# ProfessorNova/PPO-Car

Measured on AMD Instinct MI355X. Metric: env steps/sec (whole node) on big_track.json, 16 rays, higher is better.
Workload: dtype f32

## Files before the change

### include/ppocar.h

```cpp
#ifndef PPOCAR_H
#define PPOCAR_H

#include <stdint.h>

#ifdef __cplusplus
extern "C" {
#endif

#define PC_OK 0
#define PC_ERR_INVALID_ARG (-1)
#define PC_ERR_IO (-2)
#define PC_ERR_PARSE (-3)
#define PC_ERR_HIP (-4)
#define PC_ERR_UNSUPPORTED (-5)
#define PC_ERR_NO_DEVICE (-6)
#define PC_ERR_TIMEOUT (-7)

#define PC_DTYPE_F32 0
#define PC_DTYPE_F64 1

typedef struct pc_track pc_track;
typedef struct pc_env pc_env;
typedef struct pc_policy pc_policy;
typedef struct pc_xchg pc_xchg;
// ... 87 lines not shown
                         uint64_t offset, const uint64_t* offset_dev, float* obs_buf, float* act_buf, float* rew_buf, float* val_buf,
                         float* term_buf, float* trunc_buf, float* logprob_buf, float* next_obs, float* next_term, float* next_trunc,
                         float* last_value, float* reward_sum, float* final_obs, int64_t slots, void* stream);

int pc_ppo_gather(int device, const int64_t* idx, int B, int D, const float* obs, const float* act, const float* logprob,
                  const float* adv, const float* ret, float* o_obs, float* o_act, float* o_logprob, float* o_adv, float* o_ret,
                  void* stream);
int pc_ppo_loss(int device, const float* logits, const float* values, const float* act, const float* old_logprob,
                const float* adv, const float* ret, int B, int A, double clip_ratio, double vf_coef, double ent_coef,
                float* dlogits, float* dvalues, float* metrics, void* stream);
int pc_clip_adam(int device, float* param, float* grad, float* exp_avg, float* exp_avg_sq, float* step_count, const float* lr_dev,
                 int64_t n, double max_norm, double grad_scale, double beta1, double beta2, double eps, void* stream);
int pc_clip_adam_advanced(int device, float* param, const float* grad, float* exp_avg, float* exp_avg_sq, const float* step_count,
                          const float* lr_dev, int64_t n, double max_norm, double grad_scale, double beta1, double beta2, double eps,
                          void* stream);

int64_t pc_ppo_workspace_floats(int B, int D, int H, int A);
int pc_ppo_minibatch(int device, const int64_t* idx, int B, int D, int H, int A, const float* obs, const float* act,
                     const float* old_logprob, const float* adv, const float* ret, float* param, float* grad, float* exp_avg,
                     float* exp_avg_sq, float* step_count, const float* lr_dev, double clip_ratio, double vf_coef, double ent_coef,
                     double max_norm, double beta1, double beta2, double eps, float* metrics, float* workspace, int apply,
                     void* stream);

int64_t pc_ppo_prepared_floats(int B, int D);
int pc_ppo_prepare(int device, const int64_t* idx, int64_t idx_ld, int n_mb, int B, int D, const float* obs, const float* act,
                   const float* old_logprob, const float* adv, const float* ret, float* prepared, void* stream);
int pc_ppo_minibatch_prepared(int device, const float* prepared_mb, int B, int D, int H, int A, float* param, float* grad, float* exp_avg,
                              float* exp_avg_sq, float* step_count, const float* lr_dev, double clip_ratio, double vf_coef,
                              double ent_coef, double max_norm, double beta1, double beta2, double eps, float* metrics,
                              float* workspace, int apply, void* stream);


#define PC_DIAG_FLOATS 8
int64_t pc_ppo_diag_workspace_floats(int B, int D, int H, int A);
int pc_ppo_minibatch_diag(int device, const int64_t* idx, int B, int D, int H, int A, const float* obs, const float* act,
                          const float* old_logprob, const float* adv, const float* ret, float* param, float* grad, float* exp_avg,
                          float* exp_avg_sq, float* step_count, const float* lr_dev, double clip_ratio, double vf_coef, double ent_coef,
                          double max_norm, double beta1, double beta2, double eps, float* metrics, float* workspace, int apply,
                          float* diag, double target_kl, void* stream);
int pc_ppo_minibatch_prepared_diag(int device, const float* prepared_mb, int B, int D, int H, int A, float* param, float* grad, float* exp_avg,
                                   float* exp_avg_sq, float* step_count, const float* lr_dev, double clip_ratio, double vf_coef,
                                   double ent_coef, double max_norm, double beta1, double beta2, double eps, float* metrics,
                                   float* workspace, int apply, float* diag, double target_kl, void* stream);
int pc_ppo_loss_diag(int device, const float* logits, const float* values, const float* act, const float* old_logprob,
                     const float* adv, const float* ret, int B, int A, double clip_ratio, double vf_coef, double ent_coef,
                     float* dlogits, float* dvalues, float* metrics, float* diag, double target_kl, void* stream);
// ... 45 lines not shown
```

### ppo-car_amd/_capi.py

```python
import ctypes as C
import os

import torch

_HERE = os.path.dirname(os.path.abspath(__file__))
_LIB_PATH = os.path.join(_HERE, "libppocar.so")

PC_OK = 0
PC_ERR_INVALID_ARG, PC_ERR_IO, PC_ERR_PARSE, PC_ERR_HIP, PC_ERR_UNSUPPORTED, PC_ERR_NO_DEVICE, PC_ERR_TIMEOUT = -1, -2, -3, -4, -5, -6, -7
PC_XCHG_HANDLE_BYTES = 128
PC_DTYPE_F32, PC_DTYPE_F64 = 0, 1
PC_EPISODE_BUFFER, PC_EPISODE_STEPS = 0, 1
PC_DIAG_FLOATS = 8
PC_TIME_LIMIT = 1000
PC_OPT_ROLLOUT_FORM, PC_OPT_ROLLOUT_EPW, PC_OPT_ROLLOUT_FAST = 1, 2, 3
PC_KERNEL_NAMES = {0: "none", 1: "K9", 2: "K9s", 3: "K9-literal", 4: "K9d-filter", 5: "K9s-literal", 6: "K9d-selector", 7: "K9m", 8: "K9m-literal"}
PC_STEP_NAMES = {0: "none", 1: "K1", 2: "K1f", 3: "K1f-table"}
DTYPES = {"f32": PC_DTYPE_F32, "float32": PC_DTYPE_F32, "f64": PC_DTYPE_F64, "float64": PC_DTYPE_F64}


class PpoCarError(RuntimeError):
    def __init__(self, code, what):
        self.code = code
        msg = f"{what}: {lib.pc_strerror(code).decode()} (code {code})"
# ... 48 lines not shown
    "pc_build_ablate": (_i, []),
    "pc_env_get_state": (_i, [_vp] * 9),
    "pc_env_set_state": (_i, [_vp] * 9),
    "pc_gae": (_i, [_i, _vp, _vp, _vp, _vp, _vp, _vp, _vp, _d, _d, _i64, _i64, _vp, _vp, _vp]),
    "pc_episode_stats": (_i, [_i, _vp, _vp, _vp, _vp, _vp, _i64, _i64, _i, _d, _vp, _vp, _vp]),
    "pc_gae_episodes": (_i, [_i, _vp, _vp, _vp, _vp, _vp, _vp, _vp, _d, _d, _i64, _i64, _vp, _vp, _d, _vp, _vp, _vp]),
    "pc_gae_bootstrap": (_i, [_i, _vp, _vp, _vp, _vp, _vp, _vp, _vp, _vp, _i64, _d, _d, _i64, _i64, _vp, _vp, _d, _vp, _vp, _vp]),
    "pc_sample": (_i, [_i, _vp, _i64, _i, C.c_uint64, C.c_uint64, _vp, _vp, _vp, _vp]),
    "pc_policy_create": (_i, [_i, _i, _i, _i, _i, _i, C.POINTER(_vp)]),
    "pc_policy_destroy": (None, [_vp]),
    "pc_policy_get": (_i, [_vp, C.POINTER(_i), C.POINTER(_i), C.POINTER(_i64)]),
    "pc_policy_pack": (_i, [_vp] + [_vp] * 8 + [_vp, _vp]),
    "pc_policy_pack_checked": (_i, [_vp] + [_vp] * 8 + [_vp, _vp, _vp]),
    "pc_policy_act": (_i, [_vp, _vp, _i64, _vp, C.c_uint64, C.c_uint64, _vp] + [_vp] * 5 + [_vp]),
    "pc_rollout": (_i, [_vp, _vp, _vp, _i64, _d, C.c_uint64, C.c_uint64, _vp] + [_vp] * 12 + [_vp]),
    "pc_rollout_final_obs": (_i, [_vp, _vp, _vp, _i64, _d, C.c_uint64, C.c_uint64, _vp] + [_vp] * 12 + [_vp, _i64, _vp]),
    "pc_env_set_option": (_i, [_vp, _i, _i]),
    "pc_env_get_option": (_i, [_vp, _i, C.POINTER(_i)]),
    "pc_ppo_gather": (_i, [_i, _vp, _i, _i] + [_vp] * 10 + [_vp]),
    "pc_ppo_loss": (_i, [_i] + [_vp] * 6 + [_i, _i, _d, _d, _d, _vp, _vp, _vp, _vp]),
    "pc_clip_adam": (_i, [_i] + [_vp] * 6 + [_i64, _d, _d, _d, _d, _d, _vp]),
    "pc_clip_adam_advanced": (_i, [_i] + [_vp] * 6 + [_i64, _d, _d, _d, _d, _d, _vp]),
    "pc_ppo_workspace_floats": (_i64, [_i, _i, _i, _i]),
    "pc_ppo_prepared_floats": (_i64, [_i, _i]),
    "pc_ppo_prepare": (_i, [_i, _vp, _i64, _i, _i, _i] + [_vp] * 5 + [_vp, _vp]),
    "pc_ppo_minibatch_prepared": (_i, [_i, _vp, _i, _i, _i, _i] + [_vp] * 6 + [_d] * 7 + [_vp, _vp, _i, _vp]),
    "pc_ppo_epoch_state_floats": (_i64, [_i, _i, _i]),
    "pc_ppo_epoch_prepared": (_i, [_i, _vp, _i, _i, _i, _i, _i] + [_vp] * 6 + [_d] * 7 + [_vp, _vp, _vp, _vp]),
    "pc_ppo_minibatch": (_i, [_i, _vp, _i, _i, _i, _i] + [_vp] * 5 + [_vp] * 6 + [_d] * 7 + [_vp, _vp, _i, _vp]),
    "pc_ppo_diag_workspace_floats": (_i64, [_i, _i, _i, _i]),
    "pc_ppo_minibatch_diag": (_i, [_i, _vp, _i, _i, _i, _i] + [_vp] * 5 + [_vp] * 6 + [_d] * 7 + [_vp, _vp, _i, _vp, _d, _vp]),
    "pc_ppo_minibatch_prepared_diag": (_i, [_i, _vp, _i, _i, _i, _i] + [_vp] * 6 + [_d] * 7 + [_vp, _vp, _i, _vp, _d, _vp]),
    "pc_ppo_loss_diag": (_i, [_i] + [_vp] * 6 + [_i, _i, _d, _d, _d, _vp, _vp, _vp, _vp, _d, _vp]),
    "pc_clip_adam_diag": (_i, [_i] + [_vp] * 6 + [_i64, _d, _d, _d, _d, _d, _vp, _vp]),
    "pc_explained_variance_workspace_doubles": (_i64, [_i]),
    "pc_explained_variance": (_i, [_i, _vp, _vp, _i64, _vp, _vp, _vp]),
    "pc_xchg_create": (_i, [_i, _i, _i, _i64, C.POINTER(_vp)]),
    "pc_xchg_local_handle": (_i, [_vp, _vp]),
    "pc_xchg_connect": (_i, [_vp, _vp]),
    "pc_xchg_connect_local": (_i, [_vp, _vp]),
    "pc_xchg_allreduce_group": (_i, [_vp, _vp, _vp]),
    "pc_xchg_set_timeout": (_i, [_vp, _d]),
    "pc_xchg_allreduce": (_i, [_vp, _vp, _vp]),
    "pc_xchg_status": (_i, [_vp]),
    "pc_xchg_destroy": (None, [_vp]),
    "pc_strerror": (C.c_char_p, [_i]),
# ... 21 lines not shown
```

### ppo-car_amd/csrc/kernels/update.hpp

```cpp
#pragma once

__global__ __launch_bounds__(256) void ppo_gather_kernel(const int64_t* __restrict__ idx, const int B, const int D,
                                                         const float* __restrict__ obs, const float* __restrict__ act,
                                                         const float* __restrict__ logprob, const float* __restrict__ adv,
                                                         const float* __restrict__ ret, float* __restrict__ o_obs,
                                                         float* __restrict__ o_act, float* __restrict__ o_logprob,
                                                         float* __restrict__ o_adv, float* __restrict__ o_ret) {
    const int W = D + 4;
    const int i = blockIdx.x * blockDim.x + threadIdx.x;
    if (i >= B * W) return;
    const int b = i / W, c = i - b * W;
    const int64_t src = idx[b];
    if (c < D) o_obs[b * D + c] = obs[src * D + c];
    else if (c == D) o_act[b] = act[src];
    else if (c == D + 1) o_logprob[b] = logprob[src];
    else if (c == D + 2) o_adv[b] = adv[src];
    else o_ret[b] = ret[src];
}

__device__ __forceinline__ float block_sum(float v, float* sh) {
    for (int m = 32; m >= 1; m >>= 1) v += __shfl_xor(v, m, 64);
    const int w = threadIdx.x >> 6, nw = (blockDim.x + 63) >> 6;
    __syncthreads();
    if ((threadIdx.x & 63) == 0) sh[w] = v;
// ... 208 lines not shown

constexpr int FB_S = 8;

struct AdamCoef { float coef, step_size, bc2_sqrt, beta1, beta2, eps; };
__device__ __forceinline__ AdamCoef adam_coef(const float norm_sq, const float step, const float lr, const float max_norm, const float beta1,
                                              const float beta2, const float eps) {
    AdamCoef c;
    c.coef = fminf(max_norm / (sqrtf(norm_sq) + 1e-6f), 1.0f);
    const float bc1 = 1.0f - powf(beta1, step), bc2 = 1.0f - powf(beta2, step);
    c.step_size = lr / bc1;
    c.bc2_sqrt = sqrtf(bc2);
    c.beta1 = beta1;
    c.beta2 = beta2;
    c.eps = eps;
    return c;
}
__device__ __forceinline__ void adam_elem(const AdamCoef& c, const float g_raw, float& p, float& m, float& v) {
    const float g = g_raw * c.coef;
    m = m + (1.0f - c.beta1) * (g - m);
    v = c.beta2 * v + (1.0f - c.beta2) * g * g;
    const float denom = sqrtf(v) / c.bc2_sqrt + c.eps;
    p = p - c.step_size * (m / denom);
}
__device__ __forceinline__ float norm_sq_from_partials(const float* __restrict__ norm_partial, const int n_norm) {
    float ss = 0.0f;
    for (int j = 0; j < n_norm; ++j) ss += norm_partial[j];
    return ss;
}
struct AdamDefer {
    const float* __restrict__ grad;
    const float* __restrict__ m_in;
    const float* __restrict__ v_in;
    float* __restrict__ p_out;
    float* __restrict__ m_out;
    float* __restrict__ v_out;
    const float* __restrict__ norm_partial;
    int n_norm;
    const float* __restrict__ step_count;
    const float* __restrict__ lr_dev;
    float max_norm, beta1, beta2, eps;
};

__device__ __forceinline__ float wave_sum(float v) {
#define PC_DPP(ctrl, rmask) v += __builtin_bit_cast(float, __builtin_amdgcn_update_dpp(0, __builtin_bit_cast(int, v), ctrl, rmask, 0xf, false))
    PC_DPP(0x111, 0xf);
    PC_DPP(0x112, 0xf);
    PC_DPP(0x114, 0xf);
    PC_DPP(0x118, 0xf);
    PC_DPP(0x142, 0xa);
    PC_DPP(0x143, 0xc);
#undef PC_DPP
    return __builtin_bit_cast(float, __builtin_amdgcn_readlane(__builtin_bit_cast(int, v), 63));
}

__device__ __forceinline__ void adv_stats(const float (&a_loc)[4], const float a_sum, const int B, float* sh, float& mean, float& sd) {
    const int u = threadIdx.x;
    mean = block_sum(a_sum, sh) * (1.0f / (float)B);
    float d2 = 0.0f;
#pragma unroll
    for (int j = 0; j < 4; ++j) {
        const int i = u + j * 256;
        const float dv = i < B ? a_loc[j] - mean : 0.0f;
        d2 += dv * dv;
    }
    sd = fmaxf(sqrtf(block_sum(d2, sh) / (float)(B - 1)), 1e-5f);
}

__global__ __launch_bounds__(256) void ppo_prepare_kernel(const int64_t* __restrict__ idx, const int64_t idx_ld, const int B, const int D,
                                                          const float* __restrict__ obs, const float* __restrict__ act,
                                                          const float* __restrict__ old_lp, const float* __restrict__ adv,
                                                          const float* __restrict__ ret, float* __restrict__ prepared,
                                                          const int64_t prep_ld) {
    __shared__ float sh[16];
    const int u = threadIdx.x;
    const int64_t* ix = idx + (int64_t)blockIdx.x * idx_ld;
    float* out = prepared + (int64_t)blockIdx.x * prep_ld;
    float* ps = out + (size_t)B * D;
    float a_loc[4], a_sum = 0.0f;
#pragma unroll
    for (int j = 0; j < 4; ++j) {
        const int i = u + j * 256;
        const int64_t src = i < B ? ix[i] : 0;
        a_loc[j] = i < B ? adv[src] : 0.0f;
        a_sum += a_loc[j];
        if (i < B) {
            ps[i] = act[src];
            ps[B + i] = old_lp[src];
            ps[2 * B + i] = a_loc[j];
            ps[3 * B + i] = ret[src];
        }
    }
    for (int i = u; i < B * D; i += 256) {
        const int b = i / D, f = i - b * D;
        out[i] = obs[ix[b] * D + f];
    }
    float mean, sd;
    adv_stats(a_loc, a_sum, B, sh, mean, sd);
    if (u == 0) {
        ps[4 * B] = mean;
        ps[4 * B + 1] = sd;
        ps[4 * B + 2] = 0.0f;
        ps[4 * B + 3] = 0.0f;
    }
}

template <int DMAX, int AC = 0, int DC = 0, bool DEFER = false, bool DIAG = false>
__device__ __forceinline__ void ppo_fwdbwd_body(const int wg, const int64_t* __restrict__ idx, const int B, const int D_rt, const int A_rt,
                                                const float* __restrict__ obs, const float* __restrict__ act,
                                                const float* __restrict__ old_lp, const float* __restrict__ adv,
                                                const float* __restrict__ ret, const float* __restrict__ param,
                                                const float clip, const float vf, const float ec,
                                                float* __restrict__ partial, float* __restrict__ metric_partial,
                                                const float* __restrict__ prep, const AdamDefer df,
                                                const float* __restrict__ diag = nullptr, float* __restrict__ diag_partial = nullptr) {
    constexpr int H = 256, S = FB_S, LDT = DMAX + 1, LDH = H + 1;
    static_assert(!(DIAG && DEFER), "the deferred chain has no diagnostics form");
    if constexpr (DIAG) if (diag[4] != 0.0f) return;
// ... 6 lines not shown
    __shared__ float sMet[S][DIAG ? 5 : 3];
    __shared__ float sSmp[S][4];
    __shared__ __attribute__((aligned(16))) float sT[H * LDT > 2 * S * LDH + 16 * LDH + 4 * S * 16 ? H * LDT : 2 * S * LDH + 16 * LDH + 4 * S * 16];
    static_assert(H * LDT >= H * DMAX + 8, "the tile holds one [H][D] block in natural order plus an alignment shift");
    float* sHid = sT;
    float* sW2 = sT + 2 * S * LDH;
    float* sP2 = sW2 + 16 * LDH;
    const int u = threadIdx.x;
    PC_STAMP_U(0)
    __syncthreads();
    const int o_aW1 = 0, o_ab1 = H * D, o_aW2 = o_ab1 + H, o_ab2 = o_aW2 + A * H, o_cW1 = o_ab2 + A, o_cb1 = o_cW1 + H * D,
              o_cW2 = o_cb1 + H, o_cb2 = o_cW2 + H, n_param = o_cb2 + 1;

    const int s0 = wg * S;
    int64_t my_src = 0;
    int64_t a_src[4] = {0, 0, 0, 0};
    if (!prep) {
        if (u < S && s0 + u < B) my_src = idx[s0 + u];
#pragma unroll
        for (int j = 0; j < 4; ++j) a_src[j] = u + j * 256 < B ? idx[u + j * 256] : 0;
    }
    const bool defer = DEFER && df.grad != nullptr;
    const bool wr = defer && wg == 0;
    float w2a[16], w2a_g[16], w2a_m[16], w2a_v[16];
#pragma unroll
    for (int o = 0; o < 16; ++o) {
        w2a[o] = o < A ? param[o_aW2 + o * H + u] : 0.0f;
        w2a_g[o] = w2a_m[o] = w2a_v[o] = 0.0f;
        if (defer && o < A) {
            w2a_g[o] = df.grad[o_aW2 + o * H + u];
            w2a_m[o] = df.m_in[o_aW2 + o * H + u];
            w2a_v[o] = df.v_in[o_aW2 + o * H + u];
        }
    }
    float w2c = param[o_cW2 + u], b1a = param[o_ab1 + u], b1c = param[o_cb1 + u];
    const int ob = u & 15;
    const int o_b2 = ob < A ? o_ab2 + ob : o_cb2;
    float b2 = ob <= A ? param[o_b2] : 0.0f;
    float sc_g[4] = {0.0f, 0.0f, 0.0f, 0.0f}, sc_m[4] = {0.0f, 0.0f, 0.0f, 0.0f}, sc_v[4] = {0.0f, 0.0f, 0.0f, 0.0f};
    const int sc_i[4] = {o_cW2 + u, o_ab1 + u, o_cb1 + u, o_b2};
    if (defer) {
#pragma unroll
        for (int q = 0; q < 4; ++q) {
            if (q < 3 || ob <= A) {
                sc_g[q] = df.grad[sc_i[q]];
                sc_m[q] = df.m_in[sc_i[q]];
// ... 8 lines not shown
#pragma unroll
    for (int net = 0; net < 2; ++net) {
        const int off = net == 0 ? o_aW1 : o_cW1, b4 = off & ~3;
        w1_shift[net] = off - b4;
        w1_b4[net] = b4;
        w1_n4[net] = (off + H * D - b4 + 3) >> 2;
        const f32x4* __restrict__ src = reinterpret_cast<const f32x4*>(param + b4);
#pragma unroll
        for (int j = 0; j < NV4; ++j) {
            const int i4 = u + 256 * j;
            const f32x4 z = {0.0f, 0.0f, 0.0f, 0.0f};
            w1raw4[net][j] = i4 < w1_n4[net] ? src[i4] : z;
            if constexpr (DEFER) {
                w1g[net][j] = w1m[net][j] = w1v[net][j] = z;
                if (defer && i4 < w1_n4[net]) {
                    w1g[net][j] = reinterpret_cast<const f32x4*>(df.grad + b4)[i4];
                    w1m[net][j] = reinterpret_cast<const f32x4*>(df.m_in + b4)[i4];
                    w1v[net][j] = reinterpret_cast<const f32x4*>(df.v_in + b4)[i4];
                }
            }
        }
    }
    if constexpr (DEFER) if (defer) {
        const AdamCoef ac = adam_coef(norm_sq_from_partials(df.norm_partial, df.n_norm), df.step_count[0], df.lr_dev[0], df.max_norm, df.beta1,
                                      df.beta2, df.eps);
#pragma unroll
        for (int o = 0; o < 16; ++o) {
            if (o < A) {
                adam_elem(ac, w2a_g[o], w2a[o], w2a_m[o], w2a_v[o]);
                if (wr) {
                    df.p_out[o_aW2 + o * H + u] = w2a[o];
                    df.m_out[o_aW2 + o * H + u] = w2a_m[o];
                    df.v_out[o_aW2 + o * H + u] = w2a_v[o];
                }
            }
        }
        float sc_p[4] = {w2c, b1a, b1c, b2};
#pragma unroll
        for (int q = 0; q < 4; ++q) {
            if (q < 3 || ob <= A) {
                adam_elem(ac, sc_g[q], sc_p[q], sc_m[q], sc_v[q]);
                if (wr && (q < 3 || u <= A)) {
                    df.p_out[sc_i[q]] = sc_p[q];
                    df.m_out[sc_i[q]] = sc_m[q];
                    df.v_out[sc_i[q]] = sc_v[q];
                }
            }
// ... 285 lines not shown
__global__ __launch_bounds__(256) void ppo_fwdbwd_kernel(const int64_t* __restrict__ idx, const int B, const int D, const int A,
                                                         const float* __restrict__ obs, const float* __restrict__ act,
                                                         const float* __restrict__ old_lp, const float* __restrict__ adv,
                                                         const float* __restrict__ ret, const float* __restrict__ param,
                                                         const float clip, const float vf, const float ec,
                                                         float* __restrict__ partial, float* __restrict__ metric_partial,
                                                         const float* __restrict__ prep, const AdamDefer df) {
    ppo_fwdbwd_body<DMAX, AC, DC, DEFER>(blockIdx.x, idx, B, D, A, obs, act, old_lp, adv, ret, param, clip, vf, ec, partial, metric_partial, prep, df);
}
template <int DMAX, int AC = 0, int DC = 0>
__global__ __launch_bounds__(256) void ppo_fwdbwd_diag_kernel(const int64_t* __restrict__ idx, const int B, const int D, const int A,
                                                              const float* __restrict__ obs, const float* __restrict__ act,
                                                              const float* __restrict__ old_lp, const float* __restrict__ adv,
                                                              const float* __restrict__ ret, const float* __restrict__ param,
                                                              const float clip, const float vf, const float ec,
                                                              float* __restrict__ partial, float* __restrict__ metric_partial,
                                                              const float* __restrict__ prep, const float* __restrict__ diag,
                                                              float* __restrict__ diag_partial) {
    ppo_fwdbwd_body<DMAX, AC, DC, false, true>(blockIdx.x, idx, B, D, A, obs, act, old_lp, adv, ret, param, clip, vf, ec, partial, metric_partial, prep,
                                               AdamDefer{}, diag, diag_partial);
}

template <bool DIAG = false>
__device__ __forceinline__ void grad_reduce_body(const int blk, const float* __restrict__ partial, const int n_part, const int n,
                                                          const int HD, const int mid_end, const int n_pad,
                                                          float* __restrict__ grad, float* __restrict__ norm_partial,
                                                          const float* __restrict__ metric_partial, const int B, const float vf,
                                                          const float ec, float* __restrict__ metrics, float* __restrict__ step_count,
                                                          float* __restrict__ diag = nullptr, const float* __restrict__ diag_partial = nullptr,
                                                          const float kl_stop = 0.0f) {
    __shared__ float sh[16];
    __syncthreads();
    float dg_val = 0.0f, flag_val = 0.0f;
    if constexpr (DIAG) {
        if ((int)threadIdx.x < 2 * n_part) dg_val = diag_partial[threadIdx.x];
        flag_val = diag[4];
    }
    const int i = blk * blockDim.x + threadIdx.x;
    const float mp_first = (blk == 0 && (int)threadIdx.x < n_part * 4) ? metric_partial[threadIdx.x] : 0.0f;
    float g = 0.0f;
    if (i < n) {
        const int pm = i < HD ? i : (i < mid_end ? i + HD : (i < mid_end + HD ? i - (mid_end - HD) : i));
        const float* __restrict__ pp = partial + pm;
        int pidx = 0;
        for (; pidx + 64 <= n_part; pidx += 64) {
            float t[64];
#pragma unroll
            for (int j = 0; j < 64; ++j) t[j] = pp[(size_t)(pidx + j) * n_pad];
#pragma unroll
            for (int j = 0; j < 64; ++j) g += t[j];
        }
        for (; pidx + 32 <= n_part; pidx += 32) {
            float t[32];
#pragma unroll
            for (int j = 0; j < 32; ++j) t[j] = pp[(size_t)(pidx + j) * n_pad];
#pragma unroll
            for (int j = 0; j < 32; ++j) g += t[j];
        }
        for (; pidx + 8 <= n_part; pidx += 8) {
            float t[8];
#pragma unroll
            for (int j = 0; j < 8; ++j) t[j] = pp[(size_t)(pidx + j) * n_pad];
#pragma unroll
            for (int j = 0; j < 8; ++j) g += t[j];
        }
        for (; pidx < n_part; ++pidx) g += pp[(size_t)pidx * n_pad];
    }
    if constexpr (DIAG) {
        __shared__ __attribute__((aligned(8))) float sDg[256];
        sDg[threadIdx.x] = dg_val;
        __syncthreads();
        if (flag_val != 0.0f) return;
        float kl = 0.0f, nc = 0.0f;
#pragma unroll 8
        for (int p = 0; p < n_part; ++p) {
            const float2 v = reinterpret_cast<const float2*>(sDg)[p];
            kl += v.x;
            nc += v.y;
        }
        const DiagSums d{kl / (float)B, nc / (float)B};
        if (blk == 0 && threadIdx.x == 0) diag_book(diag, d, kl_stop);
        if (kl_stop > 0.0f && d.kl > kl_stop) return;
    }
    if (i < n) grad[i] = g;
    const float ss = block_sum(g * g, sh);
    if (threadIdx.x == 0) norm_partial[blk] = ss;
    if (blk == 0) {
        __shared__ float sMp[256];
        float mt[3] = {0.0f, 0.0f, 0.0f};
        for (int p0 = 0; p0 < n_part; p0 += 64) {
            __syncthreads();
            sMp[threadIdx.x] = p0 == 0 ? mp_first : (p0 * 4 + (int)threadIdx.x < n_part * 4 ? metric_partial[p0 * 4 + threadIdx.x] : 0.0f);
            __syncthreads();
            if (threadIdx.x < 3) {
                float mv[64];
#pragma unroll
                for (int pidx = 0; pidx < 64; ++pidx) mv[pidx] = sMp[pidx * 4 + threadIdx.x];
#pragma unroll
                for (int pidx = 0; pidx < 64; ++pidx) mt[threadIdx.x] += mv[pidx];
            }
        }
        if (threadIdx.x < 3) sh[threadIdx.x] = mt[threadIdx.x] / (float)B;
        __syncthreads();
        if (threadIdx.x == 0) {
            metrics[0] += sh[0];
            metrics[1] += sh[1];
            metrics[2] += sh[2];
            metrics[3] += sh[0] + vf * sh[1] - ec * sh[2];
            if (step_count) step_count[0] += 1.0f;
        }
    }
}

__global__ __launch_bounds__(256) void grad_reduce_kernel(const float* __restrict__ partial, const int n_part, const int n,
                                                          const int HD, const int mid_end, const int n_pad,
                                                          float* __restrict__ grad, float* __restrict__ norm_partial,
                                                          const float* __restrict__ metric_partial, const int B, const float vf,
                                                          const float ec, float* __restrict__ metrics, float* __restrict__ step_count) {
    grad_reduce_body(blockIdx.x, partial, n_part, n, HD, mid_end, n_pad, grad, norm_partial, metric_partial, B, vf, ec, metrics, step_count);
}
__global__ __launch_bounds__(256) void grad_reduce_diag_kernel(const float* __restrict__ partial, const int n_part, const int n,
                                                               const int HD, const int mid_end, const int n_pad,
                                                               float* __restrict__ grad, float* __restrict__ norm_partial,
                                                               const float* __restrict__ metric_partial, const int B, const float vf,
                                                               const float ec, float* __restrict__ metrics, float* __restrict__ step_count,
                                                               float* __restrict__ diag, const float* __restrict__ diag_partial,
                                                               const float kl_stop) {
    grad_reduce_body<true>(blockIdx.x, partial, n_part, n, HD, mid_end, n_pad, grad, norm_partial, metric_partial, B, vf, ec, metrics, step_count,
                           diag, diag_partial, kl_stop);
}

template <bool DIAG = false>
__device__ __forceinline__ void adam_body(const int blk, const float* __restrict__ p_in, const float* __restrict__ m_in, const float* __restrict__ v_in,
                                          float* __restrict__ grad, float* __restrict__ p_out, float* __restrict__ m_out, float* __restrict__ v_out,
                                          const float* __restrict__ step_count, const float* __restrict__ lr_dev,
                                          const float* __restrict__ norm_partial, const int n_norm, const int n, const float max_norm,
                                          const float beta1, const float beta2, const float eps, const float* __restrict__ diag = nullptr) {
    __shared__ float sNorm[256];
    const int i = blk * blockDim.x + threadIdx.x;
    const bool live = i < n;
    const float g_raw = live ? grad[i] : 0.0f;
    float m = live ? m_in[i] : 0.0f, v = live ? v_in[i] : 0.0f, p = live ? p_in[i] : 0.0f;
    const float step = step_count[0], lr = lr_dev[0];
    float flag = 0.0f;
    if constexpr (DIAG) flag = diag[4];
    float ss = 0.0f;
    for (int j0 = 0; j0 < n_norm; j0 += 256) {
        __syncthreads();
        if (j0 + (int)threadIdx.x < n_norm) sNorm[threadIdx.x] = norm_partial[j0 + threadIdx.x];
        __syncthreads();
        const int cnt = n_norm - j0 < 256 ? n_norm - j0 : 256;
        for (int j = 0; j < cnt; ++j) ss += sNorm[j];
    }
    const AdamCoef ac = adam_coef(ss, step, lr, max_norm, beta1, beta2, eps);
    if (!live) return;
    if constexpr (DIAG) if (flag != 0.0f) return;
    grad[i] = g_raw * ac.coef;
    adam_elem(ac, g_raw, p, m, v);
    m_out[i] = m;
    v_out[i] = v;
    p_out[i] = p;
}

__global__ __launch_bounds__(256) void adam_kernel(const float* __restrict__ p_in, const float* __restrict__ m_in, const float* __restrict__ v_in,
                                                   float* __restrict__ grad, float* __restrict__ p_out, float* __restrict__ m_out,
                                                   float* __restrict__ v_out, const float* __restrict__ step_count,
                                                   const float* __restrict__ lr_dev, const float* __restrict__ norm_partial,
                                                   const int n_norm, const int n, const float max_norm, const float beta1,
                                                   const float beta2, const float eps) {
    adam_body(blockIdx.x, p_in, m_in, v_in, grad, p_out, m_out, v_out, step_count, lr_dev, norm_partial, n_norm, n, max_norm, beta1, beta2, eps);
}
__global__ __launch_bounds__(256) void adam_diag_kernel(const float* __restrict__ p_in, const float* __restrict__ m_in, const float* __restrict__ v_in,
                                                        float* __restrict__ grad, float* __restrict__ p_out, float* __restrict__ m_out,
                                                        float* __restrict__ v_out, const float* __restrict__ step_count,
                                                        const float* __restrict__ lr_dev, const float* __restrict__ norm_partial,
                                                        const int n_norm, const int n, const float max_norm, const float beta1,
                                                        const float beta2, const float eps, const float* __restrict__ diag) {
    adam_body<true>(blockIdx.x, p_in, m_in, v_in, grad, p_out, m_out, v_out, step_count, lr_dev, norm_partial, n_norm, n, max_norm, beta1, beta2, eps, diag);
}


__global__ __launch_bounds__(256) void clip_adam_mb_kernel(float* __restrict__ param, float* __restrict__ grad, float* __restrict__ exp_avg,
                                                           float* __restrict__ exp_avg_sq, const float* __restrict__ step_count,
                                                           const float* __restrict__ lr_dev, const int n, const float max_norm,
                                                           const float grad_scale, const float beta1, const float beta2, const float eps) {
    __shared__ float sh[16];
    const int i = blockIdx.x * blockDim.x + threadIdx.x;
    const bool live = i < n;
    const float g_own = live ? grad[i] * grad_scale : 0.0f, m0 = live ? exp_avg[i] : 0.0f, v0 = live ? exp_avg_sq[i] : 0.0f;
    const float p0 = live ? param[i] : 0.0f;
    const float step = step_count[0], lr = lr_dev[0];
    float ss = 0.0f;
    const bool vec = (reinterpret_cast<uintptr_t>(grad) & 15) == 0;
    const int n4 = vec ? n >> 2 : 0;
    const float4* __restrict__ g4 = reinterpret_cast<const float4*>(grad);
    for (int j0 = threadIdx.x; j0 < n4; j0 += 16 * 256) {
        float4 t[16];
#pragma unroll
        for (int q = 0; q < 16; ++q) t[q] = j0 + 256 * q < n4 ? g4[j0 + 256 * q] : make_float4(0.0f, 0.0f, 0.0f, 0.0f);
#pragma unroll
        for (int q = 0; q < 16; ++q) {
// ... 14 lines not shown
```

### ppo-car_amd/csrc/ppocar.hip

```cpp
#include <hip/hip_runtime.h>

#include <algorithm>
#include <atomic>
#include <cmath>
#include <cstdio>
#include <cstdlib>
#include <cstring>
#include <memory>
#include <new>
#include <string>
#include <tuple>
#include <unordered_map>
#include <unordered_set>
#include <climits>
#include <utility>
#include <vector>

#include "ppocar_internal.h"

#include "kernels/env_math.hpp"
#include "kernels/env_step.hpp"
#include "kernels/gae_sample.hpp"
#include "kernels/policy.hpp"
#include "kernels/rollout.hpp"
// ... 1588 lines not shown
    DeviceGuard guard(e->device);
    if (!guard.ok) return PC_ERR_NO_DEVICE;
    const RolloutIO io{image, p->A, (int)T, reward_scale, seed, offset, offset_dev, obs_buf, act_buf, rew_buf, val_buf, term_buf, trunc_buf, logprob_buf,
                       next_obs, next_term, next_trunc, last_value, reward_sum, final_obs};
    rc = plan.launch(e, plan, io, stream);
    if (rc != PC_OK) return rc;
    e->last_kernel = plan.kernel;
    return PC_OK;
}

int64_t pc_ppo_workspace_floats(int B, int D, int H, int A) {
    g_hip_err.clear();
    if (H != 256 || A < 1 || A > 15 || D < 1 || D > 40 || B < 2 || B > 1024) return PC_ERR_UNSUPPORTED;
    const int64_t n_param = 2 * ((int64_t)H * D + H) + (int64_t)A * H + A + H + 1;
    const int64_t n_part = (B + FB_S - 1) / FB_S;
    return n_part * ((n_param + 3) & ~(int64_t)3) + n_part * 4 + (n_param + 255) / 256;
}

int64_t pc_ppo_diag_workspace_floats(int B, int D, int H, int A) {
    const int64_t base = pc_ppo_workspace_floats(B, D, H, A);
    return base < 0 ? base : base + 2 * (int64_t)((B + FB_S - 1) / FB_S);
}

struct MbPlan {
    int n_param, n_part, n_blk, n_pad, HD, mid_end;
    float *partial, *metric_partial, *norm_partial, *diag_partial;
    MbPlan(int B, int D, int H, int A, float* workspace) {
        n_param = 2 * (H * D + H) + A * H + A + H + 1;
        n_part = (B + FB_S - 1) / FB_S;
        n_blk = (n_param + 255) / 256;
        n_pad = (n_param + 3) & ~3;
        HD = H * D;
        mid_end = HD + H + A * H + A;
        partial = workspace;
        metric_partial = partial + (size_t)n_part * n_pad;
        norm_partial = metric_partial + n_part * 4;
        diag_partial = norm_partial + n_blk;
    }
};

static void launch_fwdbwd(const MbPlan& pl, const int64_t* idx, const float* prep, int B, int D, int A, const float* obs, const float* act,
                          const float* old_logprob, const float* adv, const float* ret, const float* param, double clip_ratio, double vf_coef,
                          double ent_coef, const AdamDefer& df, hipStream_t st) {
#define PC_FB(DM, ACV, DCV, DF)                                                                                          \
    hipLaunchKernelGGL((ppo_fwdbwd_kernel<DM, ACV, DCV, DF>), dim3(pl.n_part), dim3(256), 0, st, idx, B, D, A, obs, act, old_logprob, adv, ret, param, \
                       (float)clip_ratio, (float)vf_coef, (float)ent_coef, pl.partial, pl.metric_partial, prep, df)
    if (A == 9 && D == 23) { if (df.grad) PC_FB(24, 9, 23, true); else PC_FB(24, 9, 23, false); }
    else if (A == 9 && D == 18) { if (df.grad) PC_FB(24, 9, 18, true); else PC_FB(24, 9, 18, false); }
    else if (A == 9 && D == 39) { if (df.grad) PC_FB(40, 9, 39, true); else PC_FB(40, 9, 39, false); }
    else if (D <= 24) PC_FB(24, 0, 0, false);
    else PC_FB(40, 0, 0, false);
#undef PC_FB
}
static void launch_fwdbwd_diag(const MbPlan& pl, const int64_t* idx, const float* prep, int B, int D, int A, const float* obs, const float* act,
                               const float* old_logprob, const float* adv, const float* ret, const float* param, double clip_ratio, double vf_coef,
                               double ent_coef, const float* diag, hipStream_t st) {
#define PC_FB(DM, ACV, DCV)                                                                                              \
    hipLaunchKernelGGL((ppo_fwdbwd_diag_kernel<DM, ACV, DCV>), dim3(pl.n_part), dim3(256), 0, st, idx, B, D, A, obs, act, old_logprob, adv, ret, param, \
                       (float)clip_ratio, (float)vf_coef, (float)ent_coef, pl.partial, pl.metric_partial, prep, diag, pl.diag_partial)
    if (A == 9 && D == 23) PC_FB(24, 9, 23);
    else if (A == 9 && D == 18) PC_FB(24, 9, 18);
    else if (A == 9 && D == 39) PC_FB(40, 9, 39);
    else if (D <= 24) PC_FB(24, 0, 0);
    else PC_FB(40, 0, 0);
#undef PC_FB
}
static bool mb_defer_shape(int D, int A) { return A == 9 && (D == 18 || D == 23 || D == 39); }

static void launch_reduce(const MbPlan& pl, int B, double vf_coef, double ent_coef, float* grad, float* metrics, float* step_count, hipStream_t st) {
    hipLaunchKernelGGL(grad_reduce_kernel, dim3(pl.n_blk), dim3(256), 0, st, pl.partial, pl.n_part, pl.n_param, pl.HD, pl.mid_end, pl.n_pad, grad,
                       pl.norm_partial, pl.metric_partial, B, (float)vf_coef, (float)ent_coef, metrics, step_count);
}

static void launch_adam(const MbPlan& pl, const float* p_in, const float* m_in, const float* v_in, float* grad, float* p_out, float* m_out,
                        float* v_out, const float* step_count, const float* lr_dev, double max_norm, double beta1, double beta2, double eps,
                        hipStream_t st) {
    hipLaunchKernelGGL(adam_kernel, dim3(pl.n_blk), dim3(256), 0, st, p_in, m_in, v_in, grad, p_out, m_out, v_out, step_count, lr_dev,
                       pl.norm_partial, pl.n_blk, pl.n_param, (float)max_norm, (float)beta1, (float)beta2, (float)eps);
}

static int ppo_minibatch_impl(int device, const int64_t* idx, const float* prep, int B, int D, int H, int A, const float* obs,
                              const float* act, const float* old_logprob, const float* adv, const float* ret, float* param, float* grad,
                              float* exp_avg, float* exp_avg_sq, float* step_count, const float* lr_dev, double clip_ratio,
                              double vf_coef, double ent_coef, double max_norm, double beta1, double beta2, double eps, float* metrics,
                              float* workspace, int apply, void* stream, float* diag = nullptr, double target_kl = 0.0) {
    if (!param || !grad || !metrics || !workspace) return PC_ERR_INVALID_ARG;
    if (!prep && (!idx || !obs || !act || !old_logprob || !adv || !ret)) return PC_ERR_INVALID_ARG;
    if (apply == 1 && (!exp_avg || !exp_avg_sq || !step_count || !lr_dev)) return PC_ERR_INVALID_ARG;
    if (apply == 2 && !step_count) return PC_ERR_INVALID_ARG;
    if (apply < 0 || apply > 2) return PC_ERR_INVALID_ARG;
    if (H != 256 || A < 1 || A > 15 || D < 1 || D > 40 || B < 2 || B > 1024) return PC_ERR_UNSUPPORTED;
    if (diag && apply == 2) return PC_ERR_UNSUPPORTED;
    if (diag && device < 0) return PC_ERR_NO_DEVICE;
    DeviceGuard guard(device);
    if (!guard.ok) return PC_ERR_NO_DEVICE;
    const MbPlan pl(B, D, H, A, workspace);
    hipStream_t st = (hipStream_t)stream;
    if (diag) {
        launch_fwdbwd_diag(pl, idx, prep, B, D, A, obs, act, old_logprob, adv, ret, param, clip_ratio, vf_coef, ent_coef, diag, st);
        hipLaunchKernelGGL(grad_reduce_diag_kernel, dim3(pl.n_blk), dim3(256), 0, st, pl.partial, pl.n_part, pl.n_param, pl.HD, pl.mid_end, pl.n_pad,
                           grad, pl.norm_partial, pl.metric_partial, B, (float)vf_coef, (float)ent_coef, metrics, apply ? step_count : nullptr, diag,
                           pl.diag_partial, kl_stop_of(target_kl));
        if (apply == 1)
            hipLaunchKernelGGL(adam_diag_kernel, dim3(pl.n_blk), dim3(256), 0, st, param, exp_avg, exp_avg_sq, grad, param, exp_avg, exp_avg_sq, step_count,
                               lr_dev, pl.norm_partial, pl.n_blk, pl.n_param, (float)max_norm, (float)beta1, (float)beta2, (float)eps, diag);
        HIPCHK(hipGetLastError());
        return PC_OK;
    }
    launch_fwdbwd(pl, idx, prep, B, D, A, obs, act, old_logprob, adv, ret, param, clip_ratio, vf_coef, ent_coef, AdamDefer{}, st);
    launch_reduce(pl, B, vf_coef, ent_coef, grad, metrics, apply ? step_count : nullptr, st);
    if (apply == 1) launch_adam(pl, param, exp_avg, exp_avg_sq, grad, param, exp_avg, exp_avg_sq, step_count, lr_dev, max_norm, beta1, beta2, eps, st);
    HIPCHK(hipGetLastError());
    return PC_OK;
}

int pc_ppo_minibatch(int device, const int64_t* idx, int B, int D, int H, int A, const float* obs, const float* act,
                     const float* old_logprob, const float* adv, const float* ret, float* param, float* grad, float* exp_avg,
                     float* exp_avg_sq, float* step_count, const float* lr_dev, double clip_ratio, double vf_coef, double ent_coef,
                     double max_norm, double beta1, double beta2, double eps, float* metrics, float* workspace, int apply,
                     void* stream) {
    g_hip_err.clear();
    return ppo_minibatch_impl(device, idx, nullptr, B, D, H, A, obs, act, old_logprob, adv, ret, param, grad, exp_avg, exp_avg_sq,
                              step_count, lr_dev, clip_ratio, vf_coef, ent_coef, max_norm, beta1, beta2, eps, metrics, workspace, apply,
                              stream);
}

int pc_ppo_minibatch_diag(int device, const int64_t* idx, int B, int D, int H, int A, const float* obs, const float* act,
                          const float* old_logprob, const float* adv, const float* ret, float* param, float* grad, float* exp_avg,
                          float* exp_avg_sq, float* step_count, const float* lr_dev, double clip_ratio, double vf_coef, double ent_coef,
                          double max_norm, double beta1, double beta2, double eps, float* metrics, float* workspace, int apply,
                          float* diag, double target_kl, void* stream) {
    g_hip_err.clear();
    if (!diag) return PC_ERR_INVALID_ARG;
    return ppo_minibatch_impl(device, idx, nullptr, B, D, H, A, obs, act, old_logprob, adv, ret, param, grad, exp_avg, exp_avg_sq,
                              step_count, lr_dev, clip_ratio, vf_coef, ent_coef, max_norm, beta1, beta2, eps, metrics, workspace, apply,
                              stream, diag, target_kl);
}

int64_t pc_ppo_prepared_floats(int B, int D) {
    g_hip_err.clear();
    if (D < 1 || D > 40 || B < 2 || B > 1024) return PC_ERR_UNSUPPORTED;
    return (int64_t)B * (D + 4) + 4;
}

int pc_ppo_prepare(int device, const int64_t* idx, int64_t idx_ld, int n_mb, int B, int D, const float* obs, const float* act,
                   const float* old_logprob, const float* adv, const float* ret, float* prepared, void* stream) {
    g_hip_err.clear();
    if (!idx || !obs || !act || !old_logprob || !adv || !ret || !prepared || n_mb < 1 || idx_ld < B) return PC_ERR_INVALID_ARG;
    if (D < 1 || D > 40 || B < 2 || B > 1024) return PC_ERR_UNSUPPORTED;
    DeviceGuard guard(device);
    if (!guard.ok) return PC_ERR_NO_DEVICE;
    hipLaunchKernelGGL(ppo_prepare_kernel, dim3(n_mb), dim3(256), 0, (hipStream_t)stream, idx, idx_ld, B, D, obs, act, old_logprob, adv, ret,
                       prepared, (int64_t)B * (D + 4) + 4);
    HIPCHK(hipGetLastError());
    return PC_OK;
}

int pc_ppo_minibatch_prepared(int device, const float* prepared_mb, int B, int D, int H, int A, float* param, float* grad, float* exp_avg,
                              float* exp_avg_sq, float* step_count, const float* lr_dev, double clip_ratio, double vf_coef,
                              double ent_coef, double max_norm, double beta1, double beta2, double eps, float* metrics,
                              float* workspace, int apply, void* stream) {
    g_hip_err.clear();
    if (!prepared_mb) return PC_ERR_INVALID_ARG;
    return ppo_minibatch_impl(device, nullptr, prepared_mb, B, D, H, A, nullptr, nullptr, nullptr, nullptr, nullptr, param, grad, exp_avg,
                              exp_avg_sq, step_count, lr_dev, clip_ratio, vf_coef, ent_coef, max_norm, beta1, beta2, eps, metrics,
                              workspace, apply, stream);
}

int pc_ppo_minibatch_prepared_diag(int device, const float* prepared_mb, int B, int D, int H, int A, float* param, float* grad, float* exp_avg,
                                   float* exp_avg_sq, float* step_count, const float* lr_dev, double clip_ratio, double vf_coef,
                                   double ent_coef, double max_norm, double beta1, double beta2, double eps, float* metrics,
                                   float* workspace, int apply, float* diag, double target_kl, void* stream) {
    g_hip_err.clear();
    if (!prepared_mb || !diag) return PC_ERR_INVALID_ARG;
    return ppo_minibatch_impl(device, nullptr, prepared_mb, B, D, H, A, nullptr, nullptr, nullptr, nullptr, nullptr, param, grad, exp_avg,
                              exp_avg_sq, step_count, lr_dev, clip_ratio, vf_coef, ent_coef, max_norm, beta1, beta2, eps, metrics,
// ... 288 lines not shown
```

Measured before the change: 3.968 billion.

## Parallelize PPO prepare gather and use wave readlane norm reduction in update

The prepare kernel now splits the observation gather for each minibatch across several workgroups, with unrolled batched index loads, plus a separate workgroup for the scalar columns and advantage stats. The gradient-norm partial sum switches from serial global loads or an LDS loop to a wave-wide load followed by readlane accumulation, with the first load issued early. The grad-reduce bookkeeping (metrics, step count) moves to an extra keeper block that reads the old values early. A runtime switch keeps the old form available. All of this targets the PPO update phase rather than env stepping, so its effect on env steps/sec depends on how much of the node time the update takes.

New measurement: 4.015 billion, median of 6. +1.2%, better.

```diff
diff --git a/include/ppocar.h b/include/ppocar.h
--- a/include/ppocar.h
+++ b/include/ppocar.h
@@ -133,6 +133,7 @@
                      double max_norm, double beta1, double beta2, double eps, float* metrics, float* workspace, int apply,
                      void* stream);
 
+int pc_ppo_update_form(int form);
 int64_t pc_ppo_prepared_floats(int B, int D);
 int pc_ppo_prepare(int device, const int64_t* idx, int64_t idx_ld, int n_mb, int B, int D, const float* obs, const float* act,
                    const float* old_logprob, const float* adv, const float* ret, float* prepared, void* stream);
diff --git a/ppo-car_amd/_capi.py b/ppo-car_amd/_capi.py
--- a/ppo-car_amd/_capi.py
+++ b/ppo-car_amd/_capi.py
@@ -94,6 +94,7 @@
     "pc_clip_adam": (_i, [_i] + [_vp] * 6 + [_i64, _d, _d, _d, _d, _d, _vp]),
     "pc_clip_adam_advanced": (_i, [_i] + [_vp] * 6 + [_i64, _d, _d, _d, _d, _d, _vp]),
     "pc_ppo_workspace_floats": (_i64, [_i, _i, _i, _i]),
+    "pc_ppo_update_form": (_i, [_i]),
     "pc_ppo_prepared_floats": (_i64, [_i, _i]),
     "pc_ppo_prepare": (_i, [_i, _vp, _i64, _i, _i, _i] + [_vp] * 5 + [_vp, _vp]),
     "pc_ppo_minibatch_prepared": (_i, [_i, _vp, _i, _i, _i, _i] + [_vp] * 6 + [_d] * 7 + [_vp, _vp, _i, _vp]),
diff --git a/ppo-car_amd/csrc/kernels/update.hpp b/ppo-car_amd/csrc/kernels/update.hpp
--- a/ppo-car_amd/csrc/kernels/update.hpp
+++ b/ppo-car_amd/csrc/kernels/update.hpp
@@ -254,9 +254,17 @@
     const float denom = sqrtf(v) / c.bc2_sqrt + c.eps;
     p = p - c.step_size * (m / denom);
 }
-__device__ __forceinline__ float norm_sq_from_partials(const float* __restrict__ norm_partial, const int n_norm) {
+__device__ __forceinline__ float norm_partials_request(const float* __restrict__ norm_partial, const int n_norm, const int j0 = 0) {
+    const int j = j0 + (int)(threadIdx.x & 63);
+    return j < n_norm ? norm_partial[j] : 0.0f;
+}
+__device__ __forceinline__ float norm_sq_from_partials(const float* __restrict__ norm_partial, const int n_norm, const float first) {
     float ss = 0.0f;
-    for (int j = 0; j < n_norm; ++j) ss += norm_partial[j];
+    for (int j0 = 0; j0 < n_norm; j0 += 64) {
+        const float mine = j0 == 0 ? first : norm_partials_request(norm_partial, n_norm, j0);
+#pragma unroll
+        for (int j = 0; j < 64; ++j) ss += __builtin_bit_cast(float, __builtin_amdgcn_readlane(__builtin_bit_cast(int, mine), j));
+    }
     return ss;
 }
 struct AdamDefer {
@@ -298,33 +306,61 @@
     sd = fmaxf(sqrtf(block_sum(d2, sh) / (float)(B - 1)), 1e-5f);
 }
 
+constexpr int PREP_ROW_WG = 8, PREP_UNROLL = 8;
 __global__ __launch_bounds__(256) void ppo_prepare_kernel(const int64_t* __restrict__ idx, const int64_t idx_ld, const int B, const int D,
                                                           const float* __restrict__ obs, const float* __restrict__ act,
                                                           const float* __restrict__ old_lp, const float* __restrict__ adv,
                                                           const float* __restrict__ ret, float* __restrict__ prepared,
-                                                          const int64_t prep_ld) {
+                                                          const int64_t prep_ld, const int row_wg) {
     __shared__ float sh[16];
     const int u = threadIdx.x;
-    const int64_t* ix = idx + (int64_t)blockIdx.x * idx_ld;
-    float* out = prepared + (int64_t)blockIdx.x * prep_ld;
+    const int per_mb = row_wg > 1 ? row_wg + 1 : 1;
+    const int mb = blockIdx.x / per_mb, part = blockIdx.x - mb * per_mb;
+    const int64_t* ix = idx + (int64_t)mb * idx_ld;
+    float* out = prepared + (int64_t)mb * prep_ld;
+    if (part < row_wg) {
+        const int n_el = B * D, per = (n_el + row_wg - 1) / row_wg;
+        const int e0 = part * per, e1 = e0 + per < n_el ? e0 + per : n_el;
+        for (int i0 = e0 + u; i0 < e1; i0 += 256 * PREP_UNROLL) {
+            int64_t src[PREP_UNROLL];
+            float val[PREP_UNROLL];
+#pragma unroll
+            for (int q = 0; q < PREP_UNROLL; ++q) {
+                const int i = i0 + 256 * q;
+                const int b = i < e1 ? i / D : 0;
+                src[q] = ix[b] * D + (i - b * D);
+            }
+#pragma unroll
+            for (int q = 0; q < PREP_UNROLL; ++q) val[q] = i0 + 256 * q < e1 ? obs[src[q]] : 0.0f;
+#pragma unroll
+            for (int q = 0; q < PREP_UNROLL; ++q)
+                if (i0 + 256 * q < e1) out[i0 + 256 * q] = val[q];
+        }
+        if (row_wg > 1) return;
+    }
     float* ps = out + (size_t)B * D;
-    float a_loc[4], a_sum = 0.0f;
+    int64_t src[4];
+#pragma unroll
+    for (int j = 0; j < 4; ++j) src[j] = ix[u + j * 256 < B ? u + j * 256 : 0];
+    float a_loc[4], s_act[4], s_lp[4], s_ret[4], a_sum = 0.0f;
+#pragma unroll
+    for (int j = 0; j < 4; ++j) {
+        a_loc[j] = adv[src[j]];
+        s_act[j] = act[src[j]];
+        s_lp[j] = old_lp[src[j]];
+        s_ret[j] = ret[src[j]];
+    }
 #pragma unroll
     for (int j = 0; j < 4; ++j) {
         const int i = u + j * 256;
-        const int64_t src = i < B ? ix[i] : 0;
-        a_loc[j] = i < B ? adv[src] : 0.0f;
+        if (i >= B) a_loc[j] = 0.0f;
         a_sum += a_loc[j];
         if (i < B) {
-            ps[i] = act[src];
-            ps[B + i] = old_lp[src];
+            ps[i] = s_act[j];
+            ps[B + i] = s_lp[j];
             ps[2 * B + i] = a_loc[j];
-            ps[3 * B + i] = ret[src];
-        }
-    }
-    for (int i = u; i < B * D; i += 256) {
-        const int b = i / D, f = i - b * D;
-        out[i] = obs[ix[b] * D + f];
+            ps[3 * B + i] = s_ret[j];
+        }
     }
     float mean, sd;
     adv_stats(a_loc, a_sum, B, sh, mean, sd);
@@ -377,6 +413,8 @@
     }
     const bool defer = DEFER && df.grad != nullptr;
     const bool wr = defer && wg == 0;
+    float norm_first = 0.0f;
+    if constexpr (DEFER) if (defer) norm_first = norm_partials_request(df.norm_partial, df.n_norm);
     float w2a[16], w2a_g[16], w2a_m[16], w2a_v[16];
 #pragma unroll
     for (int o = 0; o < 16; ++o) {
@@ -431,7 +469,7 @@
         }
     }
     if constexpr (DEFER) if (defer) {
-        const AdamCoef ac = adam_coef(norm_sq_from_partials(df.norm_partial, df.n_norm), df.step_count[0], df.lr_dev[0], df.max_norm, df.beta1,
+        const AdamCoef ac = adam_coef(norm_sq_from_partials(df.norm_partial, df.n_norm, norm_first), df.step_count[0], df.lr_dev[0], df.max_norm, df.beta1,
                                       df.beta2, df.eps);
 #pragma unroll
         for (int o = 0; o < 16; ++o) {
@@ -763,7 +801,7 @@
 }
 
 template <bool DIAG = false>
-__device__ __forceinline__ void grad_reduce_body(const int blk, const float* __restrict__ partial, const int n_part, const int n,
+__device__ __forceinline__ void grad_reduce_body(const int blk, const int n_blk, const int keeper_blk, const float* __restrict__ partial, const int n_part, const int n,
                                                           const int HD, const int mid_end, const int n_pad,
                                                           float* __restrict__ grad, float* __restrict__ norm_partial,
                                                           const float* __restrict__ metric_partial, const int B, const float vf,
@@ -777,10 +815,17 @@
         if ((int)threadIdx.x < 2 * n_part) dg_val = diag_partial[threadIdx.x];
         flag_val = diag[4];
     }
+    const bool keeper = blk == keeper_blk, slice = blk < n_blk;
     const int i = blk * blockDim.x + threadIdx.x;
-    const float mp_first = (blk == 0 && (int)threadIdx.x < n_part * 4) ? metric_partial[threadIdx.x] : 0.0f;
+    const float mp_first = (keeper && (int)threadIdx.x < n_part * 4) ? metric_partial[threadIdx.x] : 0.0f;
+    float m_old[4] = {0.0f, 0.0f, 0.0f, 0.0f}, step_old = 0.0f;
+    if (keeper && threadIdx.x == 0) {
+#pragma unroll
+        for (int q = 0; q < 4; ++q) m_old[q] = metrics[q];
+        if (step_count) step_old = step_count[0];
+    }
     float g = 0.0f;
-    if (i < n) {
+    if (slice && i < n) {
         const int pm = i < HD ? i : (i < mid_end ? i + HD : (i < mid_end + HD ? i - (mid_end - HD) : i));
         const float* __restrict__ pp = partial + pm;
         int pidx = 0;
@@ -820,13 +865,15 @@
             nc += v.y;
         }
         const DiagSums d{kl / (float)B, nc / (float)B};
-        if (blk == 0 && threadIdx.x == 0) diag_book(diag, d, kl_stop);
+        if (keeper && threadIdx.x == 0) diag_book(diag, d, kl_stop);
         if (kl_stop > 0.0f && d.kl > kl_stop) return;
     }
-    if (i < n) grad[i] = g;
-    const float ss = block_sum(g * g, sh);
-    if (threadIdx.x == 0) norm_partial[blk] = ss;
-    if (blk == 0) {
+    if (slice) {
+        if (i < n) grad[i] = g;
+        const float ss = block_sum(g * g, sh);
+        if (threadIdx.x == 0) norm_partial[blk] = ss;
+    }
+    if (keeper) {
         __shared__ float sMp[256];
         float mt[3] = {0.0f, 0.0f, 0.0f};
         for (int p0 = 0; p0 < n_part; p0 += 64) {
@@ -844,11 +891,11 @@
         if (threadIdx.x < 3) sh[threadIdx.x] = mt[threadIdx.x] / (float)B;
         __syncthreads();
         if (threadIdx.x == 0) {
-            metrics[0] += sh[0];
-            metrics[1] += sh[1];
-            metrics[2] += sh[2];
-            metrics[3] += sh[0] + vf * sh[1] - ec * sh[2];
-            if (step_count) step_count[0] += 1.0f;
+            metrics[0] = m_old[0] + sh[0];
+            metrics[1] = m_old[1] + sh[1];
+            metrics[2] = m_old[2] + sh[2];
+            metrics[3] = m_old[3] + (sh[0] + vf * sh[1] - ec * sh[2]);
+            if (step_count) step_count[0] = step_old + 1.0f;
         }
     }
 }
@@ -857,8 +904,9 @@
                                                           const int HD, const int mid_end, const int n_pad,
                                                           float* __restrict__ grad, float* __restrict__ norm_partial,
                                                           const float* __restrict__ metric_partial, const int B, const float vf,
-                                                          const float ec, float* __restrict__ metrics, float* __restrict__ step_count) {
-    grad_reduce_body(blockIdx.x, partial, n_part, n, HD, mid_end, n_pad, grad, norm_partial, metric_partial, B, vf, ec, metrics, step_count);
+                                                          const float ec, float* __restrict__ metrics, float* __restrict__ step_count,
+                                                          const int n_blk, const int keeper_blk) {
+    grad_reduce_body(blockIdx.x, n_blk, keeper_blk, partial, n_part, n, HD, mid_end, n_pad, grad, norm_partial, metric_partial, B, vf, ec, metrics, step_count);
 }
 __global__ __launch_bounds__(256) void grad_reduce_diag_kernel(const float* __restrict__ partial, const int n_part, const int n,
                                                                const int HD, const int mid_end, const int n_pad,
@@ -866,8 +914,8 @@
                                                                const float* __restrict__ metric_partial, const int B, const float vf,
                                                                const float ec, float* __restrict__ metrics, float* __restrict__ step_count,
                                                                float* __restrict__ diag, const float* __restrict__ diag_partial,
-                                                               const float kl_stop) {
-    grad_reduce_body<true>(blockIdx.x, partial, n_part, n, HD, mid_end, n_pad, grad, norm_partial, metric_partial, B, vf, ec, metrics, step_count,
+                                                               const float kl_stop, const int n_blk, const int keeper_blk) {
+    grad_reduce_body<true>(blockIdx.x, n_blk, keeper_blk, partial, n_part, n, HD, mid_end, n_pad, grad, norm_partial, metric_partial, B, vf, ec, metrics, step_count,
                            diag, diag_partial, kl_stop);
 }
 
@@ -876,22 +924,29 @@
                                           float* __restrict__ grad, float* __restrict__ p_out, float* __restrict__ m_out, float* __restrict__ v_out,
                                           const float* __restrict__ step_count, const float* __restrict__ lr_dev,
                                           const float* __restrict__ norm_partial, const int n_norm, const int n, const float max_norm,
-                                          const float beta1, const float beta2, const float eps, const float* __restrict__ diag = nullptr) {
-    __shared__ float sNorm[256];
+                                          const float beta1, const float beta2, const float eps, const int lds_norm,
+                                          const float* __restrict__ diag = nullptr) {
     const int i = blk * blockDim.x + threadIdx.x;
     const bool live = i < n;
+    const float norm_first = norm_partials_request(norm_partial, n_norm);
     const float g_raw = live ? grad[i] : 0.0f;
     float m = live ? m_in[i] : 0.0f, v = live ? v_in[i] : 0.0f, p = live ? p_in[i] : 0.0f;
     const float step = step_count[0], lr = lr_dev[0];
     float flag = 0.0f;
     if constexpr (DIAG) flag = diag[4];
-    float ss = 0.0f;
-    for (int j0 = 0; j0 < n_norm; j0 += 256) {
-        __syncthreads();
-        if (j0 + (int)threadIdx.x < n_norm) sNorm[threadIdx.x] = norm_partial[j0 + threadIdx.x];
-        __syncthreads();
-        const int cnt = n_norm - j0 < 256 ? n_norm - j0 : 256;
-        for (int j = 0; j < cnt; ++j) ss += sNorm[j];
+    float ss;
+    if (lds_norm) {
+        __shared__ float sNorm[256];
+        ss = 0.0f;
+        for (int j0 = 0; j0 < n_norm; j0 += 256) {
+            __syncthreads();
+            if (j0 + (int)threadIdx.x < n_norm) sNorm[threadIdx.x] = norm_partial[j0 + threadIdx.x];
+            __syncthreads();
+            const int cnt = n_norm - j0 < 256 ? n_norm - j0 : 256;
+            for (int j = 0; j < cnt; ++j) ss += sNorm[j];
+        }
+    } else {
+        ss = norm_sq_from_partials(norm_partial, n_norm, norm_first);
     }
     const AdamCoef ac = adam_coef(ss, step, lr, max_norm, beta1, beta2, eps);
     if (!live) return;
@@ -908,16 +963,18 @@
                                                    float* __restrict__ v_out, const float* __restrict__ step_count,
                                                    const float* __restrict__ lr_dev, const float* __restrict__ norm_partial,
                                                    const int n_norm, const int n, const float max_norm, const float beta1,
-                                                   const float beta2, const float eps) {
-    adam_body(blockIdx.x, p_in, m_in, v_in, grad, p_out, m_out, v_out, step_count, lr_dev, norm_partial, n_norm, n, max_norm, beta1, beta2, eps);
+                                                   const float beta2, const float eps, const int lds_norm) {
+    adam_body(blockIdx.x, p_in, m_in, v_in, grad, p_out, m_out, v_out, step_count, lr_dev, norm_partial, n_norm, n, max_norm, beta1, beta2, eps, lds_norm);
 }
 __global__ __launch_bounds__(256) void adam_diag_kernel(const float* __restrict__ p_in, const float* __restrict__ m_in, const float* __restrict__ v_in,
                                                         float* __restrict__ grad, float* __restrict__ p_out, float* __restrict__ m_out,
                                                         float* __restrict__ v_out, const float* __restrict__ step_count,
                                                         const float* __restrict__ lr_dev, const float* __restrict__ norm_partial,
                                                         const int n_norm, const int n, const float max_norm, const float beta1,
-                                                        const float beta2, const float eps, const float* __restrict__ diag) {
-    adam_body<true>(blockIdx.x, p_in, m_in, v_in, grad, p_out, m_out, v_out, step_count, lr_dev, norm_partial, n_norm, n, max_norm, beta1, beta2, eps, diag);
+                                                        const float beta2, const float eps, const int lds_norm,
+                                                        const float* __restrict__ diag) {
+    adam_body<true>(blockIdx.x, p_in, m_in, v_in, grad, p_out, m_out, v_out, step_count, lr_dev, norm_partial, n_norm, n, max_norm, beta1, beta2, eps,
+                    lds_norm, diag);
 }
 
 
diff --git a/ppo-car_amd/csrc/ppocar.hip b/ppo-car_amd/csrc/ppocar.hip
--- a/ppo-car_amd/csrc/ppocar.hip
+++ b/ppo-car_amd/csrc/ppocar.hip
@@ -1634,6 +1634,12 @@
     return base < 0 ? base : base + 2 * (int64_t)((B + FB_S - 1) / FB_S);
 }
 
+static std::atomic<int> g_update_form{0};
+int pc_ppo_update_form(int form) {
+    if (form == 0 || form == 1) return g_update_form.exchange(form);
+    return g_update_form.load();
+}
+
 struct MbPlan {
     int n_param, n_part, n_blk, n_pad, HD, mid_end;
     float *partial, *metric_partial, *norm_partial, *diag_partial;
@@ -1680,15 +1686,17 @@
 static bool mb_defer_shape(int D, int A) { return A == 9 && (D == 18 || D == 23 || D == 39); }
 
 static void launch_reduce(const MbPlan& pl, int B, double vf_coef, double ent_coef, float* grad, float* metrics, float* step_count, hipStream_t st) {
-    hipLaunchKernelGGL(grad_reduce_kernel, dim3(pl.n_blk), dim3(256), 0, st, pl.partial, pl.n_part, pl.n_param, pl.HD, pl.mid_end, pl.n_pad, grad,
-                       pl.norm_partial, pl.metric_partial, B, (float)vf_coef, (float)ent_coef, metrics, step_count);
+    const bool old_form = g_update_form.load() == 1;
+    hipLaunchKernelGGL(grad_reduce_kernel, dim3(pl.n_blk + (old_form ? 0 : 1)), dim3(256), 0, st, pl.partial, pl.n_part, pl.n_param, pl.HD, pl.mid_end,
+                       pl.n_pad, grad, pl.norm_partial, pl.metric_partial, B, (float)vf_coef, (float)ent_coef, metrics, step_count, pl.n_blk,
+                       old_form ? 0 : pl.n_blk);
 }
 
 static void launch_adam(const MbPlan& pl, const float* p_in, const float* m_in, const float* v_in, float* grad, float* p_out, float* m_out,
                         float* v_out, const float* step_count, const float* lr_dev, double max_norm, double beta1, double beta2, double eps,
                         hipStream_t st) {
     hipLaunchKernelGGL(adam_kernel, dim3(pl.n_blk), dim3(256), 0, st, p_in, m_in, v_in, grad, p_out, m_out, v_out, step_count, lr_dev,
-                       pl.norm_partial, pl.n_blk, pl.n_param, (float)max_norm, (float)beta1, (float)beta2, (float)eps);
+                       pl.norm_partial, pl.n_blk, pl.n_param, (float)max_norm, (float)beta1, (float)beta2, (float)eps, g_update_form.load());
 }
 
 static int ppo_minibatch_impl(int device, const int64_t* idx, const float* prep, int B, int D, int H, int A, const float* obs,
@@ -1710,12 +1718,14 @@
     hipStream_t st = (hipStream_t)stream;
     if (diag) {
         launch_fwdbwd_diag(pl, idx, prep, B, D, A, obs, act, old_logprob, adv, ret, param, clip_ratio, vf_coef, ent_coef, diag, st);
-        hipLaunchKernelGGL(grad_reduce_diag_kernel, dim3(pl.n_blk), dim3(256), 0, st, pl.partial, pl.n_part, pl.n_param, pl.HD, pl.mid_end, pl.n_pad,
+        const bool old_form = g_update_form.load() == 1;
+        hipLaunchKernelGGL(grad_reduce_diag_kernel, dim3(pl.n_blk + (old_form ? 0 : 1)), dim3(256), 0, st, pl.partial, pl.n_part, pl.n_param, pl.HD, pl.mid_end, pl.n_pad,
                            grad, pl.norm_partial, pl.metric_partial, B, (float)vf_coef, (float)ent_coef, metrics, apply ? step_count : nullptr, diag,
-                           pl.diag_partial, kl_stop_of(target_kl));
+                           pl.diag_partial, kl_stop_of(target_kl), pl.n_blk, old_form ? 0 : pl.n_blk);
         if (apply == 1)
             hipLaunchKernelGGL(adam_diag_kernel, dim3(pl.n_blk), dim3(256), 0, st, param, exp_avg, exp_avg_sq, grad, param, exp_avg, exp_avg_sq, step_count,
-                               lr_dev, pl.norm_partial, pl.n_blk, pl.n_param, (float)max_norm, (float)beta1, (float)beta2, (float)eps, diag);
+                               lr_dev, pl.norm_partial, pl.n_blk, pl.n_param, (float)max_norm, (float)beta1, (float)beta2, (float)eps,
+                               old_form ? 1 : 0, diag);
         HIPCHK(hipGetLastError());
         return PC_OK;
     }
@@ -1762,8 +1772,9 @@
     if (D < 1 || D > 40 || B < 2 || B > 1024) return PC_ERR_UNSUPPORTED;
     DeviceGuard guard(device);
     if (!guard.ok) return PC_ERR_NO_DEVICE;
-    hipLaunchKernelGGL(ppo_prepare_kernel, dim3(n_mb), dim3(256), 0, (hipStream_t)stream, idx, idx_ld, B, D, obs, act, old_logprob, adv, ret,
-                       prepared, (int64_t)B * (D + 4) + 4);
+    const int row_wg = g_update_form.load() == 1 ? 1 : PREP_ROW_WG;
+    hipLaunchKernelGGL(ppo_prepare_kernel, dim3(n_mb * (row_wg > 1 ? row_wg + 1 : 1)), dim3(256), 0, (hipStream_t)stream, idx, idx_ld, B, D, obs, act,
+                       old_logprob, adv, ret, prepared, (int64_t)B * (D + 4) + 4, row_wg);
     HIPCHK(hipGetLastError());
     return PC_OK;
 }
```
